# alessioGalatolo/GAN-2D-to-3D

Hardware: AMD Instinct MI355X
Metric: GAN2Shape step iters/sec, faces 128×128 b=8, 1/2/4/8 MI355X (higher is better)
Workload: dtype f32; 1 GPU; face128_n8; image_size=128, gan_size=128, n_proj_samples=8, mfma_operands=f32, prior=ellipsoid, step_mix=7:7:6 (step1:step2:step3, main.py:148 stage 0), images_per_rank=1

## Files before the change

gan-2d-to-3d_amd/csrc/conv_wgrad_core.h:

```cpp
#pragma once
#include <algorithm>
#include "g2s_common.h"

namespace g2s {

typedef float wg_f32x16 __attribute__((ext_vector_type(16)));

constexpr int WG_BM = 64, WG_BN = 64, WG_BK = 32, WG_THREADS = 256;
constexpr int WG_E = WG_BM * WG_BK / WG_THREADS;

struct WgradParams {
    const float *A, *G;
    float *dw;
    int B, Ca, Cg, PH, PW, GH, GW, k, stride, pad;
    int N;
    int K;
    int ktiles;
    int per;
    int atomic;
    int groups;
};

__device__ __forceinline__ void wgrad_block(const WgradParams &p, float (&As)[WG_BK][WG_BM + 1],
                                            float (&Bs)[WG_BK][WG_BN + 1], const int bx, const int by,
                                            const int bz) {
    const int tid = threadIdx.x, lane = tid & 63, wave = tid >> 6;
    const int wm = wave >> 1, wn = wave & 1, l31 = lane & 31, lk = lane >> 5;
    const int tiles_m = (p.Ca + WG_BM - 1) / WG_BM;
    const int m0 = (bx % tiles_m) * WG_BM, n0 = (bx / tiles_m) * WG_BN;
    const int kt0 = by * p.per, kt1 = min(p.ktiles, kt0 + p.per);
    const int P = p.PH * p.PW, KK = p.k * p.k;
    const int grp = bz;
    const int Ca_tot = p.Ca * p.groups, Cg_tot = p.Cg * p.groups;

    const int kl = tid & 31, r0 = tid >> 5;
    int gbase[WG_E], dy[WG_E], dx[WG_E];
    bool nok[WG_E], aok[WG_E];
#pragma unroll
    for (int e = 0; e < WG_E; e++) {
        const int n = n0 + r0 + 8 * e;
        nok[e] = n < p.N;
        const int g = n / KK, t = n - g * KK;
        gbase[e] = g * p.GH * p.GW;
        dy[e] = t / p.k - p.pad;
        dx[e] = t % p.k - p.pad;
        aok[e] = m0 + r0 + 8 * e < p.Ca;
    }
    float ra[WG_E], rb[WG_E];
    auto load = [&](int kt) {
        const int kg = kt * WG_BK + kl;
        const bool kok = kg < p.K;
        const int b = kok ? kg / P : 0, pix = kok ? kg - b * P : 0;
        const int py = pix / p.PW, px = pix - py * p.PW;
        const float *ap = p.A + ((size_t)b * Ca_tot + grp * p.Ca + m0 + r0) * P + pix;
        const float *gp = p.G + ((size_t)b * Cg_tot + grp * p.Cg) * p.GH * p.GW;
        const int gy0 = py * p.stride, gx0 = px * p.stride;
#pragma unroll
        for (int e = 0; e < WG_E; e++) {
            ra[e] = (kok && aok[e]) ? ap[(size_t)8 * e * P] : 0.0f;
            const int gy = gy0 + dy[e], gx = gx0 + dx[e];
            const bool ok = kok && nok[e] && gy >= 0 && gy < p.GH && gx >= 0 && gx < p.GW;
            rb[e] = ok ? gp[gbase[e] + gy * p.GW + gx] : 0.0f;
        }
    };
    wg_f32x16 acc;
#pragma unroll
    for (int r = 0; r < 16; r++) acc[r] = 0.0f;
    if (kt0 < kt1) load(kt0);
    for (int kt = kt0; kt < kt1; kt++) {
        __syncthreads();
#pragma unroll
        for (int e = 0; e < WG_E; e++) {
            As[kl][r0 + 8 * e] = ra[e];
            Bs[kl][r0 + 8 * e] = rb[e];
        }
        __syncthreads();
        if (kt + 1 < kt1) load(kt + 1);
#pragma unroll
        for (int k2 = 0; k2 < WG_BK; k2 += 2) {
            const float a = As[k2 + lk][wm * 32 + l31];
            const float b = Bs[k2 + lk][wn * 32 + l31];
            acc = __builtin_amdgcn_mfma_f32_32x32x2f32(a, b, acc, 0, 0, 0);
        }
    }
    const int n = n0 + wn * 32 + l31;
// ... 51 lines not shown
```

gan-2d-to-3d_amd/csrc/modconv.hip:

```cpp
#include "modconv_desc.h"
#include "conv_wgrad_core.h"
#include "thinconv.h"
#include "xcd_tile.h"

namespace g2s {

template <int T> struct KTile {
    static constexpr int BKT = (T == 9) ? 18 : (T == 25) ? 26 : 16;
    static constexpr int CPT = BKT / T;
    static constexpr int KMAX = (T == 25) ? 26 : 18;
};

template <int BM, int BN, int T, bool PARTIAL, bool SCALE>
__device__ __forceinline__ void modconv_body(const ConvDesc &d, const ConvClass &c,
                                             float (&As)[2][KTile<T>::KMAX][BM + 1],
                                             float (&Bs)[2][KTile<T>::KMAX + 1][BN],
                                             const int (&stab)[25], const int tile_id, const int grp,
                                             const int kt_begin, const int kt_end, const bool atomic) {
    constexpr int BKT = KTile<T>::BKT, CPT = KTile<T>::CPT, BK_MAX = KTile<T>::KMAX;
    constexpr int WAVES_M = BM >= 64 ? 2 : 1, WAVES_N = 4 / WAVES_M;
    constexpr int WMT = BM / (32 * WAVES_M), WNT = BN / (32 * WAVES_N);
    constexpr bool WIDE = (T == 9);
    constexpr int EA = WIDE ? (BM * 6 + NTHREADS - 1) / NTHREADS : (BM * BKT + NTHREADS - 1) / NTHREADS;
    constexpr int EB = (BN * BKT + NTHREADS - 1) / NTHREADS;
    const int tid = threadIdx.x, lane = tid & 63, wave = tid >> 6;
    const int wm = wave / WAVES_N, wn = wave % WAVES_N;
    const int Ncls = d.B * c.OH * c.OW;
    const int tiles_m = (d.M + BM - 1) / BM;
    const int m0 = (tile_id % tiles_m) * BM;
    const int n0 = (tile_id / tiles_m) * BN;
    const int HW = d.H * d.W;
    constexpr int OOB = 0x7fffffff;

    const auto rx = __builtin_amdgcn_make_buffer_rsrc((void *)(d.x + (size_t)grp * d.Cr * HW), 0,
                                                      (d.B * d.Cx - grp * d.Cr) * HW * 4, 0x00020000);
    const auto rw = __builtin_amdgcn_make_buffer_rsrc((void *)(d.w + (size_t)grp * (d.w_bytes / 4)), 0, d.w_bytes, 0x00020000);
    const auto rsc = __builtin_amdgcn_make_buffer_rsrc(
        (void *)(SCALE ? d.in_scale : d.w), 0, SCALE ? d.B * d.Cr * 4 : 4, 0x00020000);

    const int nB = tid % BN;
    const int ng = n0 + nB;
    const bool n_ok = ng < Ncls;
    int bb = 0, iy0 = 0, ix0 = 0;
    if (n_ok) {
        bb = ng / (c.OH * c.OW);
        const int r = ng % (c.OH * c.OW);
        iy0 = (r / c.OW) * d.is;
        ix0 = (r % c.OW) * d.is;
    }
    int offB[EB], dchB[EB];
#pragma unroll
    for (int e = 0; e < EB; e++) {
        const int k = tid / BN + e * (NTHREADS / BN);
        const int dch = k / T, t = k - dch * T;
        const int tb = stab[t < T ? t : 0];
        const int iy = iy0 + (tb & 0xff) - 8, ix = ix0 + ((tb >> 8) & 0xff) - 8;
        const bool ok = n_ok && k < BKT && dch < CPT && iy >= 0 && iy < d.H && ix >= 0 && ix < d.W;
        offB[e] = ok ? (((bb * d.Cx + dch) * d.H + iy) * d.W + ix) * 4 : OOB;
        dchB[e] = dch;
    }
    const int offS = n_ok ? bb * d.Cr * 4 : OOB;
    int offA[EA], ldsA[EA], dchA[EA];
#pragma unroll
    for (int e = 0; e < EA; e++) {
        const int idx = tid + e * NTHREADS;
        if (WIDE) {
            const int m = idx / 6, r = idx % 6, dch = r / 3, tg = r % 3;
            const bool in = idx < BM * 6, ok = in && m0 + m < d.M;
            offA[e] = ok ? ((m0 + m) * d.w_ms + dch * d.w_ks + 3 * tg) * 4 : OOB;
            ldsA[e] = in ? (dch * 9 + 3 * tg) * (BM + 1) + m : BM;
            dchA[e] = dch;
        } else {
            const int k = idx % BKT, m = idx / BKT;
            const int dch = k / T, t = k - dch * T;
            const bool ok = idx < BM * BKT && dch < CPT && m0 + m < d.M;
            offA[e] = ok ? ((m0 + m) * d.w_ms + dch * d.w_ks + (stab[t] >> 16)) * 4 : OOB;
            ldsA[e] = (idx < BM * BKT) ? k * (BM + 1) + m : BM;
            dchA[e] = dch;
        }
    }

    float ra[EA][WIDE ? 3 : 1], rb[EB];
    float rs[WIDE ? 2 : EB], rsn[2];
    auto loadA = [&](int e, int kt) {
        const int ch0 = kt * CPT;
        const int vo = (PARTIAL && dchA[e] >= d.Cr - ch0) ? OOB : offA[e];
        if constexpr (WIDE) {
            const u32x3 v = __builtin_amdgcn_raw_buffer_load_b96(rw, vo, ch0 * d.w_ks * 4, 0);
            ra[e][0] = __uint_as_float(v.x);
            ra[e][1] = __uint_as_float(v.y);
            ra[e][2] = __uint_as_float(v.z);
        } else {
            ra[e][0] = __uint_as_float(__builtin_amdgcn_raw_buffer_load_b32(rw, vo, ch0 * d.w_ks * 4, 0));
        }
    };
    auto loadB = [&](int e, int kt) {
        const int ch0 = kt * CPT;
        const bool out = PARTIAL && dchB[e] >= d.Cr - ch0;
        rb[e] = __uint_as_float(__builtin_amdgcn_raw_buffer_load_b32(rx, out ? OOB : offB[e], ch0 * HW * 4, 0));
        if constexpr (SCALE && !WIDE)
            rs[e] = __uint_as_float(__builtin_amdgcn_raw_buffer_load_b32(
                rsc, out ? OOB : offS + dchB[e] * 4, ch0 * 4, 0));
    };
    auto loadS = [&](int kt, float (&dst)[2]) {
        if constexpr (SCALE && WIDE) {
            const int ch0 = kt * CPT;
            dst[0] = __uint_as_float(__builtin_amdgcn_raw_buffer_load_b32(rsc, offS, ch0 * 4, 0));
            dst[1] = __uint_as_float(__builtin_amdgcn_raw_buffer_load_b32(
                rsc, (PARTIAL && 1 >= d.Cr - ch0) ? OOB : offS + 4, ch0 * 4, 0));
        }
    };
    auto storeA = [&](int e, float *abuf) {
        if constexpr (WIDE) {
            abuf[ldsA[e]] = ra[e][0];
            abuf[ldsA[e] + (BM + 1)] = ra[e][1];
            abuf[ldsA[e] + 2 * (BM + 1)] = ra[e][2];
        } else {
            abuf[ldsA[e]] = ra[e][0];
        }
    };
    auto storeB = [&](int e, float (*bbuf)[BN]) {
        const int k = tid / BN + e * (NTHREADS / BN);
        float v = rb[e];
        if constexpr (SCALE) v *= WIDE ? (dchB[e] ? rs[1] : rs[0]) : rs[e];
        bbuf[k < BKT ? k : BK_MAX][nB] = v;
    };

    f32x16 acc[WMT][WNT];
#pragma unroll
    for (int i = 0; i < WMT; i++)
#pragma unroll
        for (int j = 0; j < WNT; j++)
#pragma unroll
            for (int r = 0; r < 16; r++) acc[i][j][r] = 0.0f;

    const int kt_last = kt_end - 1;
#pragma unroll
    for (int e = 0; e < EA; e++) loadA(e, kt_begin);
#pragma unroll
    for (int e = 0; e < EB; e++) loadB(e, kt_begin);
    if constexpr (WIDE) loadS(kt_begin, rs);
#pragma unroll
    for (int e = 0; e < EA; e++) { storeA(e, &As[0][0][0]); loadA(e, min(kt_begin + 1, kt_last)); }
#pragma unroll
    for (int e = 0; e < EB; e++) { storeB(e, Bs[0]); loadB(e, min(kt_begin + 1, kt_last)); }
    if constexpr (WIDE) loadS(min(kt_begin + 1, kt_last), rs);
    __syncthreads();
// ... 62 lines not shown
#pragma unroll
        for (int i = 0; i < WMT; i++)
#pragma unroll
            for (int r = 0; r < 16; r++) {
                const int m = m0 + wm * (BM / WAVES_M) + i * 32 + (r & 3) + 8 * (r >> 2) + 4 * lk;
                if (m >= d.M) continue;
                float v = acc[i][j][r];
                if (ob) v *= ob[m];
                if (gbias) v += gbias[m];
                v += nz;
                if (d.act) v = (v > 0.0f ? v : v * d.act_alpha) * d.act_gain;
                float *dst = yb + (size_t)m * d.OHf * d.OWf;
                if (atomic) unsafeAtomicAdd(dst, v);
                else *dst = v;
            }
    }
}

static __host__ __device__ inline int ktiles_of(int Cr, int T) {
    const int cpt = (T == 9) ? 2 : (T == 25) ? 1 : 16 / T;
    return (Cr + cpt - 1) / cpt;
}

template <int BM, int BN, int KMAX>
__device__ __forceinline__ void modconv_segment(const ConvDesc &d, const ConvClass &c,
                                                float (&As)[2][KMAX][BM + 1], float (&Bs)[2][KMAX + 1][BN],
                                                const int (&stab)[25], const int tile_id, const int grp,
                                                const int kb, const int ke, const bool atomic) {
    const bool scale = d.in_scale != nullptr;
#define G2S_BODY(T, PART, SC) modconv_body<BM, BN, T, PART, SC>(d, c, As, Bs, stab, tile_id, grp, kb, ke, atomic)
#define G2S_TAPS(T, CPT)                                   \
    if (d.Cr % CPT) {                                      \
        if (scale) G2S_BODY(T, true, true);                \
        else G2S_BODY(T, true, false);                     \
    } else {                                               \
        if (scale) G2S_BODY(T, false, true);               \
        else G2S_BODY(T, false, false);                    \
    }
    if constexpr (KMAX == 26) {
        G2S_BODY(25, true, false);
    } else {
        switch (c.T) {
        case 9: G2S_TAPS(9, 2) break;
        case 16: G2S_BODY(16, true, false); break;
        case 4: G2S_TAPS(4, 4) break;
        case 2: G2S_TAPS(2, 8) break;
        default: G2S_TAPS(1, 16) break;
        }
    }
#undef G2S_TAPS
#undef G2S_BODY
}

template <int BM, int BN, int KMAX>
__device__ __forceinline__ void modconv_block(const ConvDesc &d, float (&As)[2][KMAX][BM + 1],
                                              float (&Bs)[2][KMAX + 1][BN], int (&stab)[25], const int nx,
                                              const int bx, const int by, const int bz, const int row) {
    const int tiles_m = (d.M + BM - 1) / BM;
    const int tile_all0 = __builtin_amdgcn_readfirstlane(xcd_logical_tile(nx, bx, row));
    const ConvClass &c = d.cls[bz];
    const int mt_all = tile_all0 % (tiles_m * d.groups);
    const int grp = __builtin_amdgcn_readfirstlane(mt_all / tiles_m);
    const int tile_id = __builtin_amdgcn_readfirstlane((tile_all0 / (tiles_m * d.groups)) * tiles_m + mt_all % tiles_m);
    if ((int)(tile_id / tiles_m) * BN >= d.B * c.OH * c.OW) return;
    const int ktiles = ktiles_of(d.Cr, c.T);
    const int slices = d.cls_splitk[bz];
    const int per = (ktiles + slices - 1) / slices;
    const int kb = by * per;
    if (by >= slices || kb >= ktiles) return;
    if (threadIdx.x < 25) stab[threadIdx.x] = c.tab[threadIdx.x];
    __syncthreads();
    modconv_segment<BM, BN, KMAX>(d, c, As, Bs, stab, tile_id, grp, kb, min(ktiles, kb + per), slices > 1);
}

template <int BM, int BN, int KMAX>
__global__ __launch_bounds__(NTHREADS) void modconv_kernel(ConvDesc d) {
    __shared__ float As[2][KMAX][BM + 1];
    __shared__ float Bs[2][KMAX + 1][BN];
    __shared__ int stab[25];
    modconv_block<BM, BN, KMAX>(d, As, Bs, stab, gridDim.x, blockIdx.x, blockIdx.y, blockIdx.z,
                                blockIdx.y + gridDim.y * blockIdx.z);
}

__global__ __launch_bounds__(NTHREADS) void conv_wgrad_rider_kernel(WgradParams p) {
    __shared__ float Wa[WG_BK][WG_BM + 1];
    __shared__ float Wb[WG_BK][WG_BN + 1];
    wgrad_block(p, Wa, Wb, blockIdx.x, blockIdx.y, blockIdx.z);
}

template <int BM, int BN, int KMAX>
__global__ __launch_bounds__(NTHREADS) void conv_bwd_kernel(ConvDesc d, WgradParams p, int nx, int ny, int n_dgrad,
                                                            int w_tiles, int w_split) {
    __shared__ float As[2][KMAX][BM + 1];
    __shared__ float Bs[2][KMAX + 1][BN];
    __shared__ int stab[25];
    __shared__ float Wa[WG_BK][WG_BM + 1];
    __shared__ float Wb[WG_BK][WG_BN + 1];
    const int lin = blockIdx.x;
    if (lin < n_dgrad) {
        const int bx = lin % nx, row = lin / nx;
        modconv_block<BM, BN, KMAX>(d, As, Bs, stab, nx, bx, row % ny, row / ny, row);
    } else {
        const int l = lin - n_dgrad;
        const int bx = l % w_tiles, r = l / w_tiles;
        wgrad_block(p, Wa, Wb, bx, r % w_split, r / w_split);
    }
}

}

using namespace g2s;

struct TunedConv { int B, Cin, Cout, H, k, mode, transpose, fused, tile, splitk; };
static const TunedConv kTuned[] = {
#include "modconv_tuned.inc"
    {0, 0, 0, 0, 0, 0, 0, 0, 0, 0}};

struct TunedConv2d { int B, Cr, M, H, k, stride, pad, adjoint, m_major, fused, groups, tile, splitk; };
static const TunedConv2d kTuned2d[] = {
#include "conv2d_tuned.inc"
    {0, 0, 0, 0, 0, 0, 0, 0, 0, 0, 0, 0, 0}};

static thread_local int g_force_tile = -1, g_force_splitk = -1;

extern "C" int g2s_modconv_tune(int tile, int splitk) {
    G2S_REQUIRE(tile >= -2 && tile <= 4 && splitk >= -1 && splitk <= 64 && splitk != 0,
                "tile must be -1 (built-in), -2 (heuristic without the tuned table) or 0..4, "
                "splitk -1 (built-in) or 1..64");
    g_force_tile = tile;
    g_force_splitk = splitk;
    return G2S_OK;
}

struct ConvGeom {
    int k, stride, pad, adjoint, m_major;
    int out_h, out_w;
};

struct WgradRider {
    WgradParams p;
    int tiles, split;
    bool dw_is_zero;
};

struct Epilogue {
    const float *bias, *noise, *noise_w;
    int act;
    float alpha, gain;
};

template <int KMAX>
static void conv_launch_tile(const ConvDesc &d, const dim3 grid, const int pick, hipStream_t st,
                             const WgradRider *rider = nullptr) {
    const int n_dgrad = grid.x * grid.y * grid.z;
#define G2S_TILE(BM_, BN_)                                                                                           \
    if (rider)                                                                                                       \
        conv_bwd_kernel<BM_, BN_, KMAX><<<n_dgrad + rider->tiles * rider->split * rider->p.groups, NTHREADS, 0, st>>>( \
            d, rider->p, grid.x, grid.y, n_dgrad, rider->tiles, rider->split);                                       \
    else                                                                                                             \
        modconv_kernel<BM_, BN_, KMAX><<<grid, NTHREADS, 0, st>>>(d)
    switch (pick) {
    case 0: modconv_kernel<128, 128, KMAX><<<grid, NTHREADS, 0, st>>>(d); break;
    case 1: modconv_kernel<128, 64, KMAX><<<grid, NTHREADS, 0, st>>>(d); break;
    case 2: G2S_TILE(64, 64); break;
    case 3: G2S_TILE(32, 128); break;
    default: G2S_TILE(64, 128); break;
    }
#undef G2S_TILE
}

static int conv_launch(const float *x, const float *w, const float *in_scale, const float *out_scale,
                       const Epilogue &ep, float *y, int B, int Cr, int M, int H, int W, const ConvGeom &g,
                       int tuned_tile, int tuned_splitk, g2s_stream_t stream, bool y_is_zero = false,
                       bool f16_operands = false, int groups = 1, const WgradRider *rider = nullptr,
                       int *plan_needs_zero = nullptr) {
    G2S_REQUIRE(plan_needs_zero || (x && w && y), "x, w, y must not be NULL");
    G2S_REQUIRE(B > 0 && Cr > 0 && M > 0 && H > 0 && W > 0, "sizes must be positive");
    const int k = g.k, s_ = g.stride, p_ = g.pad, KK = k * k;
    G2S_REQUIRE(k >= 1 && k <= 5, "kernel size must be 1..5 (got %d)", k);
    G2S_REQUIRE(s_ == 1 || s_ == 2, "stride must be 1 or 2 (got %d)", s_);
    G2S_REQUIRE(p_ >= 0 && p_ < k, "padding must be in [0, k)");
    ConvDesc d{};
    d.x = x;
    d.w = w;
    d.in_scale = in_scale;
    d.out_scale = out_scale;
    d.bias = ep.bias;
    d.noise = ep.noise;
    d.noise_w = ep.noise_w;
    G2S_REQUIRE(!d.noise || (!f16_operands && groups == 1), "the noise epilogue exists for the fp32 kernel only");
    d.act = ep.act;
// ... 65 lines not shown
        G2S_REQUIRE(!(in_scale && T > 9), "input scales are limited to kernels of up to 3x3");
        big = big || T == 25;
    }
    long nmax = 0;
    int kt_min = 1 << 30;
    for (int i = 0; i < d.ncls; i++) {
        nmax = std::max(nmax, (long)B * d.cls[i].OH * d.cls[i].OW);
        kt_min = std::min(kt_min, ktiles_of(d.Cr, d.cls[i].T));
    }
    G2S_REQUIRE(nmax < (1l << 30) && (long)B * d.Cx * H * W < (1l << 29) && (long)groups * M * Cr * KK < (1l << 29),
                "problem too large for 32-bit byte offsets");
    hipStream_t st = as_stream(stream);
    const int cfgs[5][2] = {{128, 128}, {128, 64}, {64, 64}, {32, 128}, {64, 128}};
    int pick = 2;
    for (int i = 0; i < 3; i++) {
        const long blocks = (long)groups * cdiv(d.M, cfgs[i][0]) * cdiv(nmax, cfgs[i][1]) * d.ncls;
        if (d.M > cfgs[i][0] / 2 && blocks >= 512) { pick = i; break; }
    }
    if (d.M <= 32 && nmax >= 1024 && !f16_operands) pick = 3;
    if (f16_operands && pick == 1) pick = 2;
    if (tuned_tile >= 0 && g_force_tile != -2) pick = tuned_tile;
    else tuned_splitk = -1;
    if (g_force_tile >= 0) pick = g_force_tile;
    const int BMv = cfgs[pick][0], BNv = cfgs[pick][1];
    const int tiles = groups * cdiv(d.M, BMv) * cdiv(nmax, BNv);
    int splitk = 1;
    while ((long)tiles * d.ncls * splitk < 512 && kt_min / (splitk * 2) >= 8 && splitk < 64) splitk *= 2;
    if (tuned_splitk > 0) splitk = tuned_splitk;
    if (g_force_splitk > 0) splitk = g_force_splitk;
    if (deterministic()) splitk = 1;
    splitk = std::max(1, std::min(splitk, kt_min));
    dim3 grid(tiles, splitk, d.ncls);
    const bool split = splitk > 1;
    const bool deferred_epilogue = split && (ep.bias != nullptr || ep.act != 0 || ep.noise != nullptr);
    if (deferred_epilogue) {
        d.bias = nullptr;
        d.noise = d.noise_w = nullptr;
        d.act = 0;
    }
    d.splitk = splitk;
    int kt_max = 1;
    for (int i = 0; i < d.ncls; i++) kt_max = std::max(kt_max, ktiles_of(d.Cr, d.cls[i].T));
    for (int i = 0; i < d.ncls; i++) {
        const int kt = ktiles_of(d.Cr, d.cls[i].T);
        d.cls_splitk[i] = std::max(1, std::min(kt, (int)(((long)splitk * kt + kt_max / 2) / kt_max)));
    }
    if (plan_needs_zero) {
        *plan_needs_zero = (split || holes) ? 1 : 0;
        return G2S_OK;
    }
    if ((split || holes) && !y_is_zero) {
        if (hipMemsetAsync(y, 0, (size_t)B * d.My * d.OHf * d.OWf * sizeof(float), st) != hipSuccess)
            return fail(G2S_ERR_LAUNCH, "hipMemsetAsync(y) failed");
    }
    if (f16_operands) {
        const int rc = modconv_f16_launch(d, grid, pick, st);
        if (rc != G2S_OK) return rc;
    } else if (rider) {
        const WgradParams &p = rider->p;
        if (p.atomic && !rider->dw_is_zero &&
            hipMemsetAsync(p.dw, 0, (size_t)p.groups * p.Ca * p.N * sizeof(float), st) != hipSuccess)
            return fail(G2S_ERR_LAUNCH, "hipMemsetAsync(dw) failed");
        if (big) conv_launch_tile<26>(d, grid, pick, st, pick >= 2 ? rider : nullptr);
        else conv_launch_tile<18>(d, grid, pick, st, pick >= 2 ? rider : nullptr);
        if (pick < 2) conv_wgrad_rider_kernel<<<dim3(rider->tiles, rider->split, p.groups), NTHREADS, 0, st>>>(p);
    } else if (big) {
        conv_launch_tile<26>(d, grid, pick, st);
    } else {
        conv_launch_tile<18>(d, grid, pick, st);
    }
    int rc = check_launch("g2s_modconv");
    if (rc != G2S_OK || !deferred_epilogue) return rc;
    if (ep.noise) {
        G2S_REQUIRE(ep.bias && ep.act == 1, "noise epilogue: needs a bias and act = 1");
        return g2s_noise_bias_act(y, ep.noise, ep.noise_w, ep.bias, y, B, d.My, d.OHf * d.OWf, ep.alpha, ep.gain,
                                  stream);
    }
    return g2s_fused_bias_act(y, ep.bias, nullptr, y, (int64_t)B * d.My * d.OHf * d.OWf,
                              (int64_t)d.OHf * d.OWf, d.My, ep.act ? 3 : 1, 0, ep.alpha,
                              ep.act ? ep.gain : 1.0f, G2S_F32, stream);
}

static int modconv_launch(const float *x, const float *w, const float *in_scale,
                          const float *out_scale, const Epilogue &ep, float *y, int B, int Cin, int Cout, int H,
                          int W, int k, int mode, int transpose, g2s_stream_t stream, bool f16_operands = false,
// ... 71 lines not shown
        for (const TunedConv2d *t = kTuned2d; t->B; ++t)
            if (t->B == B && t->Cr == Cr && t->M == M && t->H == H && t->k == k && t->stride == stride &&
                t->pad == pad && t->adjoint == g.adjoint && t->m_major == g.m_major &&
                t->fused == (bias != nullptr || act != 0) && t->groups == groups) {
                tile = t->tile;
                splitk = t->splitk;
                break;
            }
    return conv_launch(x, w, nullptr, nullptr, Epilogue{bias, nullptr, nullptr, act, alpha, gain}, y, B, Cr, M, H, W,
                       g, tile, splitk, stream, y_is_zero != 0, false, groups, rider);
}

extern "C" int g2s_conv2d(const float *x, const float *w, const float *bias, float *y, int B, int Cr, int M, int H,
                          int W, int k, int stride, int pad, int adjoint, int w_m_major, int out_h, int out_w, int act,
                          float alpha, float gain, int y_is_zero, int groups, g2s_stream_t stream) {
    return conv2d_impl(x, w, bias, y, B, Cr, M, H, W, k, stride, pad, adjoint, w_m_major, out_h, out_w, act, alpha,
                       gain, y_is_zero, groups, stream);
}

extern "C" int g2s_conv2d_bwd(const float *gy, const float *w, float *gx, int B, int Cr, int M, int H, int W, int k,
                              int stride, int pad, int adjoint, int w_m_major, int out_h, int out_w, int gx_is_zero,
                              const float *A, const float *G, float *dw, int Ca, int Cg, int PH, int PW, int GH,
                              int GW, int dw_is_zero, int groups, g2s_stream_t stream) {
    WgradRider rider;
    const int rc = wgrad_plan(A, G, dw, B, Ca, Cg, PH, PW, GH, GW, k, stride, pad, groups, rider.p, rider.tiles,
                              rider.split);
    if (rc != G2S_OK) return rc;
    rider.dw_is_zero = dw_is_zero != 0;
    return conv2d_impl(gy, w, nullptr, gx, B, Cr, M, H, W, k, stride, pad, adjoint, w_m_major, out_h, out_w, 0, 0.0f,
                       1.0f, gx_is_zero, groups, stream, &rider);
}
```

gan-2d-to-3d_amd/lib.py:

```python
import ctypes as C
import os

import torch

_HERE = os.path.dirname(os.path.abspath(__file__))
LIB_PATH = os.path.join(_HERE, "lib", "libg2s.so")

G2S_F32, G2S_F16 = 0, 1
CONV_PLAIN, CONV_UP2, CONV_DOWN2 = 0, 1, 2

_lib = None

_p, _i, _f, _sz, _i64, _d = C.c_void_p, C.c_int, C.c_float, C.c_size_t, C.c_int64, C.c_double
SIGNATURES = {
    "g2s_abi_version": (_i, []),
    "g2s_last_error": (C.c_char_p, []),
    "g2s_clamp": (_i, [_p, _p, _p, _i64, _f, _f, _i, _p]),
    "g2s_avg_pyramid": (_i, [_p, _p, _i, _i64, _i, _i, _p]),
    "g2s_res_split_fwd": (_i, [_p, _p, _p, _i64, _i, _i, _p]),
    "g2s_res_split_bwd": (_i, [_p, _p, _p, _p, _i64, _i, _i, _p]),
    "g2s_depth_head_fwd": (_i, [_p, _p, _p, _i64, _i, _f, _f, _i, _f, _p]),
    "g2s_depth_head_bwd": (_i, [_p, _p, _p, _p, _p, _i64, _i, _f, _f, _i, _f, _i, _p]),
    "g2s_grid_sample_fwd": (_i, [_p, _p, _p, _i, _i, _i, _i, _i, _i, _i, _f, _f, _p]),
    "g2s_grid_sample_bwd_workspace_bytes": (_sz, [_i, _i, _i, _i]),
# ... 16 lines not shown
    "g2s_noise_bias_act": (_i, [_p, _p, _p, _p, _p, _i, _i, _i, _f, _f, _p]),
    "g2s_upfirdn2d": (_i, [_p, _p, _p] + [_i] * 14 + [_p]),
    "g2s_modconv": (_i, [_p] * 8 + [_i] * 9 + [_f, _f, _i, _p]),
    "g2s_modconv_needs_zero": (_i, [_i, _i, _i, _i, _i, _i, _i, _i, _i, _i]),
    "g2s_upfirdn2d_nba": (_i, [_p, _p, _p] + [_i] * 12 + [_p, _p, _p, _f, _f, _p]),
    "g2s_synth_bwd_rows": (_i, [_p] * 13 + [_i, _i, _i, _f, _f, _p]),
    "g2s_channel_sum": (_i, [_p, _p, _i, _i, _i, _p]),
    "g2s_demod_fwd_multi": (_i, [_p, _p, _p, _p, _p, _i, _i, _f, _p]),
    "g2s_demod_bwd_multi": (_i, [_p, _p, _p, _p, _p, _p, _p, _i, _i, _p]),
    "g2s_modconv_f16": (_i, [_p, _p, _p, _p, _p, _p, _i, _i, _i, _i, _i, _i, _i, _i, _i, _f, _f, _p]),
    "g2s_modconv_tune": (_i, [_i, _i]),
    "g2s_mfma_probe": (_i, [_p, _i, _i, _i, _p]),
    "g2s_mfma_lds_probe": (_i, [_p, _i, _i, _i, _i, _p]),
    "g2s_wino_weights_floats": (_sz, [_i, _i]),
    "g2s_wino4_weights_floats": (_sz, [_i, _i]),
    "g2s_wino4_weights": (_i, [_p, _p, _i, _i, _i, _p]),
    "g2s_wino4_supported": (_i, [_i] * 5),
    "g2s_conv3x3_wino4": (_i, [_p] * 8 + [_i] * 6 + [_f, _f, _i, _p, _i64, _p]),
    "g2s_wino_weights": (_i, [_p, _p, _i, _i, _i, _p]),
    "g2s_conv3x3_wino": (_i, [_p] * 8 + [_i] * 6 + [_f, _f, _i, _p, _i64, _p]),
    "g2s_conv2d": (_i, [_p, _p, _p, _p] + [_i] * 12 + [_i, _f, _f, _i, _i, _p]),
    "g2s_conv2d_wgrad": (_i, [_p, _p, _p] + [_i] * 10 + [_i, _i, _p]),
    "g2s_conv2d_bwd": (_i, [_p, _p, _p] + [_i] * 13 + [_p, _p, _p] + [_i] * 8 + [_p]),
    "g2s_adam_chunk": (_i64, []),
    "g2s_adam_step": (_i, [_p, _p, _p, _i, _i, _f, _f, _f, _f, _f, _p]),
    "g2s_rows_dot_scale": (_i, [_p, _p, _p, _p, _p, _p, _i, _i, _p]),
    "g2s_demod_fwd": (_i, [_p, _p, _p, _i, _i, _i, _f, _p]),
    "g2s_demod_bwd": (_i, [_p, _p, _p, _p, _p, _i, _i, _i, _p]),
    "g2s_demod_bwd_add": (_i, [_p, _p, _p, _p, _p, _p, _i, _i, _i, _p]),
    "g2s_lpips_layer_fwd": (_i, [_p, _p, _p, _p, _i, _i, _i, _p]),
    "g2s_lpips_layer_bwd": (_i, [_p, _p, _p, _p, _p, _i, _i, _i, _p]),
    "g2s_lpips_layer_bwd_ex": (_i, [_p, _p, _p, _p, _p, _i, _p, _i, _i, _i, _p]),
    "g2s_weighted_l1_fwd": (_i, [_p, _p, _p, _p, _i, _i, _i, _p]),
    "g2s_weighted_l1_bwd": (_i, [_p, _p, _p, _p, _p, _i, _i, _i, _p]),
    "g2s_weighted_l1_fwd2": (_i, [_p, _p, _p, _p, _i, _i, _i, _p]),
    "g2s_weighted_l1_bwd3": (_i, [_p] * 7 + [_f, _p, _p, _f, _f, _p, _i, _i, _i, _p]),
    "g2s_weighted_l1_bwd2": (_i, [_p, _p, _p, _p, _p, _p, _p, _i, _i, _i, _p]),
    "g2s_view_transform_fwd": (_i, [_p, _f, _f, _f, _p, _p, _i, _p]),
    "g2s_view_transform_bwd": (_i, [_p, _f, _f, _f, _p, _p, _p, _i, _p]),
    "g2s_warp_verts_fwd": (_i, [_p, _p, _p, _p, _f, _p, _i, _i, _p]),
    "g2s_warp_verts_bwd": (_i, [_p, _p, _p, _p, _f, _p, _p, _i, _i, _i, _p]),
    "g2s_inv_warp_grid_fwd": (_i, [_p, _p, _p, _p, _p, _f, _p, _i, _i, _i, _p]),
    "g2s_inv_warp_grid_bwd": (_i, [_p, _p, _p, _p, _p, _f, _p, _p, _p, _i, _i, _i, _i, _p]),
    "g2s_normal_fwd": (_i, [_p, _p, _p, _i, _i, _i, _p]),
    "g2s_normal_bwd": (_i, [_p, _p, _p, _p, _i, _i, _i, _p]),
    "g2s_shading_fwd": (_i, [_p, _p, _p, _p, _p, _i, _i, _i, _i, _p]),
# ... 74 lines not shown
```

gan-2d-to-3d_amd/op/conv.py:

```python
import torch
from torch.autograd import Function

from gan2shape_amd import lib as _lib
from gan2shape_amd import zeropool


class PassArena:

    LIMIT = 1 << 20

    def __init__(self, device, fwd_elems):
        self.device = device
        self.fwd = zeropool.zeros(fwd_elems, device) if fwd_elems else None
        self.fwd_off = 0
        self.bwd_need = 0
        self.bwd = None
        self.bwd_off = 0

    @staticmethod
    def _pad(n):
        return (n + 63) & ~63

    def take_fwd(self, shape):
        n = 1
# ... 64 lines not shown


def _conv_bwd_raw(gy, w, x, cin, cout, k, stride, pad, transposed, gx_out=None, gw_out=None, groups=1):
    B, _, H, W = gy.shape
    oh, ow = x.shape[2], x.shape[3]
    adjoint = not transposed
    gx = gx_out if gx_out is not None else torch.empty((B, groups * cin, oh, ow), dtype=torch.float32, device=gy.device)
    A, G = (x, gy) if transposed else (gy, x)
    Ca, Cg = A.shape[1] // groups, G.shape[1] // groups
    dw = gw_out if gw_out is not None else torch.empty((groups * Ca, Cg, k, k), dtype=torch.float32, device=gy.device)
    L = _lib.load()
    from gan2shape_amd.modconv import profiled
    sp = H * W if adjoint else oh * ow
    flop = 2.0 * B * groups * cout * cin * k * k * sp + 2.0 * B * groups * Ca * Cg * k * k * A.shape[2] * A.shape[3]
    with profiled(flop, 4.0 * (2 * gy.numel() + w.numel() + gx.numel() + x.numel() + dw.numel())):
        _lib.check(L.g2s_conv2d_bwd(_lib.ptr(gy), _lib.ptr(w), _lib.ptr(gx), B, cout, cin, H, W, k, stride, pad,
                                    int(adjoint), int(transposed), oh if adjoint else 0, ow if adjoint else 0,
                                    int(gx_out is not None), _lib.ptr(A), _lib.ptr(G), _lib.ptr(dw), Ca, Cg,
                                    A.shape[2], A.shape[3], G.shape[2], G.shape[3], int(gw_out is not None),
                                    groups, _lib.stream()))
    return gx, dw


class ConvFunction(Function):

    @staticmethod
    def forward(ctx, x, w, bias, stride, pad, transposed, slope, arena=None, groups=1):
        _lib.require_cuda(x, w, bias)
        if x.dtype != torch.float32 or w.dtype != torch.float32:
            raise RuntimeError("conv: float32 only")
        x, w = x.contiguous(), w.contiguous()
        k = w.shape[2]
        cin, cout = (w.shape[0] // groups, w.shape[1]) if transposed else (w.shape[1], w.shape[0] // groups)
        if x.shape[1] != groups * cin:
            raise RuntimeError(f"conv: input has {x.shape[1]} channels, weight expects {groups * cin}")
        if groups != 1 and bias is not None:
            raise RuntimeError("grouped conv: no bias")
        b = None if bias is None else bias.contiguous()
        out = None
        if arena is not None:
            oh, ow = _out_size(x.shape[2], x.shape[3], k, stride, pad, transposed)
            out = arena.take_fwd((x.shape[0], groups * cout, oh, ow))
            if ctx.needs_input_grad[0]:
                arena.reserve_bwd(x.numel())
            if ctx.needs_input_grad[1]:
                arena.reserve_bwd(w.numel())
        y = _conv2d_raw(x, w, b, cin, cout, k, stride, pad, transposed, not transposed, None,
                        slope is not None, slope or 0.0, out=out, groups=groups)
        ctx.save_for_backward(x, w, y if slope is not None else None)
        ctx.cfg = (stride, pad, transposed, slope, bias is not None, groups)
        ctx.arena = arena
        return y

    @staticmethod
    def backward(ctx, gy):
        x, w, y = ctx.saved_tensors
        stride, pad, transposed, slope, has_bias, groups = ctx.cfg
        k = w.shape[2]
        gy = gy.contiguous()
        if slope is not None:
            from gan2shape_amd.plugins import fused
            gy = fused.fused_bias_act(gy, gy.new_empty(0), y, 3, 1, float(slope), 1.0)
        cin, cout = (w.shape[0] // groups, w.shape[1]) if transposed else (w.shape[1], w.shape[0] // groups)
        gx = gw = gb = None
        arena = ctx.arena
        if ctx.needs_input_grad[0] and ctx.needs_input_grad[1]:
            gx_out = None if arena is None else arena.take_bwd(tuple(x.shape))
            gw_out = None if arena is None else arena.take_bwd(tuple(w.shape))
            gx, gw = _conv_bwd_raw(gy, w, x, cin, cout, k, stride, pad, transposed, gx_out, gw_out, groups)
        elif ctx.needs_input_grad[0]:
            out = None if arena is None else arena.take_bwd(tuple(x.shape))
            gx = _conv2d_raw(gy, w, None, cout, cin, k, stride, pad, not transposed, transposed,
                             (x.shape[2], x.shape[3]), False, 0.0, out=out, groups=groups)
        elif ctx.needs_input_grad[1]:
            out = None if arena is None else arena.take_bwd(tuple(w.shape))
            gw = (_wgrad(x, gy, k, stride, pad, out, groups) if transposed
                  else _wgrad(gy, x, k, stride, pad, out, groups))
        if has_bias and ctx.needs_input_grad[2]:
            gb = torch.empty(gy.shape[1], dtype=torch.float32, device=gy.device)
            _lib.check(_lib.load().g2s_channel_sum(_lib.ptr(gy), _lib.ptr(gb), gy.shape[0], gy.shape[1],
                                                   gy.shape[2] * gy.shape[3], _lib.stream()))
        return gx, gw, gb, None, None, None, None, None, None
# ... 43 lines not shown
```

include/g2s.h:

```cpp
#ifndef G2S_H
#define G2S_H

#include <stddef.h>
#include <stdint.h>

#ifdef __cplusplus
extern "C" {
#endif

#define G2S_ABI_VERSION 1

#define G2S_OK 0
#define G2S_ERR_INVALID (-1)
#define G2S_ERR_LAUNCH (-2)
#define G2S_ERR_WORKSPACE (-3)

#define G2S_F32 0
#define G2S_F16 1

typedef void *g2s_stream_t;

int g2s_abi_version(void);
const char *g2s_last_error(void);

// ... 83 lines not shown



#define G2S_CONV_PLAIN 0
#define G2S_CONV_UP2 1
#define G2S_CONV_DOWN2 2

int g2s_modconv(const float *x, const float *w, const float *in_scale, const float *out_scale, const float *bias,
                const float *noise, const float *noise_w, float *y, int B, int Cin, int Cout, int H, int W, int k,
                int mode, int transpose, int act, float alpha, float gain, int y_is_zero, g2s_stream_t stream);
int g2s_modconv_needs_zero(int B, int Cin, int Cout, int H, int W, int k, int mode, int transpose,
                           int has_scales, int fused);

int g2s_conv2d(const float *x, const float *w, const float *bias, float *y, int B, int Cr, int M, int H,
               int W, int k, int stride, int pad, int adjoint, int w_m_major, int out_h, int out_w,
               int act, float alpha, float gain, int y_is_zero, int groups, g2s_stream_t stream);
int g2s_conv2d_wgrad(const float *A, const float *G, float *dw, int B, int Ca, int Cg, int PH, int PW,
                     int GH, int GW, int k, int stride, int pad, int dw_is_zero, int groups, g2s_stream_t stream);

int g2s_conv2d_bwd(const float *gy, const float *w, float *gx, int B, int Cr, int M, int H, int W, int k,
                   int stride, int pad, int adjoint, int w_m_major, int out_h, int out_w, int gx_is_zero,
                   const float *A, const float *G, float *dw, int Ca, int Cg, int PH, int PW, int GH, int GW,
                   int dw_is_zero, int groups, g2s_stream_t stream);

#define G2S_ADAM_MAX_TENSORS 128
typedef struct g2s_adam_tensor {
    float *p, *m, *v;
    int64_t n;
    float *step;
    int *ticket;
} g2s_adam_tensor;
int64_t g2s_adam_chunk(void);
int g2s_adam_step(const g2s_adam_tensor *tensors, const int *chunk0, const float *const *grads, int n_tensors,
                  int n_chunks, float lr, float beta1, float beta2, float eps, float weight_decay,
                  g2s_stream_t stream);

int g2s_modconv_f16(const float *x, const float *w, const float *in_scale, const float *out_scale,
                    const float *bias, float *y, int B, int Cin, int Cout, int H, int W, int k, int mode,
                    int transpose, int act, float alpha, float gain, g2s_stream_t stream);

size_t g2s_wino_weights_floats(int M, int Cr);
int g2s_wino_weights(const float *w, float *U, int Cout, int Cin, int transpose, g2s_stream_t stream);
int g2s_conv3x3_wino(const float *x, const float *U, const float *in_scale, const float *out_scale,
                     const float *bias, const float *noise, const float *noise_w, float *y, int B, int Cr, int M,
                     int H, int W, int act, float alpha, float gain, int splitk, float *ws, int64_t ws_floats,
                     g2s_stream_t stream);
// ... 105 lines not shown
```

Before: 206.2 iters/s.

## Fuse conv backward (leaky-ReLU gate, dgrad, wgrad, bias grad) into one launch

Adds g2s_conv2d_layer_bwd, which applies the leaky-ReLU gradient gate inline while loading gy in the dgrad, wgrad and new bias-reduction blocks, all dispatched from a single conv_bwd_kernel launch. It replaces the separate fused_bias_act gate pass, the materialized gated gy, and separate bias-grad work in ConvFunction.backward, which is enabled by default. In exchange the gate reference is re-read inside each sub-kernel, small-tile picks are forced to a rider-capable tile, and bias grads use atomics when sliced.

Measured after the change: 201.1 iters/s. 2.5% lower.

```diff
diff --git a/gan-2d-to-3d_amd/csrc/conv_wgrad_core.h b/gan-2d-to-3d_amd/csrc/conv_wgrad_core.h
--- a/gan-2d-to-3d_amd/csrc/conv_wgrad_core.h
+++ b/gan-2d-to-3d_amd/csrc/conv_wgrad_core.h
@@ -21,9 +21,13 @@
     int groups;
 };
 
+__device__ __forceinline__ float gate_factor(const float ref, const float slope) { return ref > 0.0f ? 1.0f : slope; }
+
+template <bool GATE = false>
 __device__ __forceinline__ void wgrad_block(const WgradParams &p, float (&As)[WG_BK][WG_BM + 1],
                                             float (&Bs)[WG_BK][WG_BN + 1], const int bx, const int by,
-                                            const int bz) {
+                                            const int bz, const float *ref = nullptr, const float slope = 0.0f,
+                                            const bool gate_g = false) {
     const int tid = threadIdx.x, lane = tid & 63, wave = tid >> 6;
     const int wm = wave >> 1, wn = wave & 1, l31 = lane & 31, lk = lane >> 5;
     const int tiles_m = (p.Ca + WG_BM - 1) / WG_BM;
@@ -52,8 +56,10 @@
         const bool kok = kg < p.K;
         const int b = kok ? kg / P : 0, pix = kok ? kg - b * P : 0;
         const int py = pix / p.PW, px = pix - py * p.PW;
-        const float *ap = p.A + ((size_t)b * Ca_tot + grp * p.Ca + m0 + r0) * P + pix;
-        const float *gp = p.G + ((size_t)b * Cg_tot + grp * p.Cg) * p.GH * p.GW;
+        const size_t ao = ((size_t)b * Ca_tot + grp * p.Ca + m0 + r0) * P + pix;
+        const size_t go = ((size_t)b * Cg_tot + grp * p.Cg) * p.GH * p.GW;
+        const float *ap = p.A + ao;
+        const float *gp = p.G + go;
         const int gy0 = py * p.stride, gx0 = px * p.stride;
 #pragma unroll
         for (int e = 0; e < WG_E; e++) {
@@ -61,6 +67,13 @@
             const int gy = gy0 + dy[e], gx = gx0 + dx[e];
             const bool ok = kok && nok[e] && gy >= 0 && gy < p.GH && gx >= 0 && gx < p.GW;
             rb[e] = ok ? gp[gbase[e] + gy * p.GW + gx] : 0.0f;
+            if constexpr (GATE) {
+                if (gate_g) {
+                    if (ok) rb[e] *= gate_factor(ref[go + gbase[e] + gy * p.GW + gx], slope);
+                } else {
+                    if (kok && aok[e]) ra[e] *= gate_factor(ref[ao + (size_t)8 * e * P], slope);
+                }
+            }
         }
     };
     wg_f32x16 acc;
diff --git a/gan-2d-to-3d_amd/csrc/modconv.hip b/gan-2d-to-3d_amd/csrc/modconv.hip
--- a/gan-2d-to-3d_amd/csrc/modconv.hip
+++ b/gan-2d-to-3d_amd/csrc/modconv.hip
@@ -11,8 +11,13 @@
     static constexpr int KMAX = (T == 25) ? 26 : 18;
 };
 
-template <int BM, int BN, int T, bool PARTIAL, bool SCALE>
-__device__ __forceinline__ void modconv_body(const ConvDesc &d, const ConvClass &c,
+struct Gate {
+    const float *ref;
+    float slope;
+};
+
+template <int BM, int BN, int T, bool PARTIAL, bool SCALE, bool GATE>
+__device__ __forceinline__ void modconv_body(const ConvDesc &d, const ConvClass &c, const Gate &gate,
                                              float (&As)[2][KTile<T>::KMAX][BM + 1],
                                              float (&Bs)[2][KTile<T>::KMAX + 1][BN],
                                              const int (&stab)[25], const int tile_id, const int grp,
@@ -37,6 +42,9 @@
     const auto rw = __builtin_amdgcn_make_buffer_rsrc((void *)(d.w + (size_t)grp * (d.w_bytes / 4)), 0, d.w_bytes, 0x00020000);
     const auto rsc = __builtin_amdgcn_make_buffer_rsrc(
         (void *)(SCALE ? d.in_scale : d.w), 0, SCALE ? d.B * d.Cr * 4 : 4, 0x00020000);
+    const auto rgate = __builtin_amdgcn_make_buffer_rsrc(
+        (void *)(GATE ? gate.ref + (size_t)grp * d.Cr * HW : d.w), 0, GATE ? (d.B * d.Cx - grp * d.Cr) * HW * 4 : 4,
+        0x00020000);
 
     const int nB = tid % BN;
     const int ng = n0 + nB;
@@ -82,6 +90,7 @@
 
     float ra[EA][WIDE ? 3 : 1], rb[EB];
     float rs[WIDE ? 2 : EB], rsn[2];
+    float rg[GATE ? EB : 1];
     auto loadA = [&](int e, int kt) {
         const int ch0 = kt * CPT;
         const int vo = (PARTIAL && dchA[e] >= d.Cr - ch0) ? OOB : offA[e];
@@ -101,6 +110,8 @@
         if constexpr (SCALE && !WIDE)
             rs[e] = __uint_as_float(__builtin_amdgcn_raw_buffer_load_b32(
                 rsc, out ? OOB : offS + dchB[e] * 4, ch0 * 4, 0));
+        if constexpr (GATE)
+            rg[e] = __uint_as_float(__builtin_amdgcn_raw_buffer_load_b32(rgate, out ? OOB : offB[e], ch0 * HW * 4, 0));
     };
     auto loadS = [&](int kt, float (&dst)[2]) {
         if constexpr (SCALE && WIDE) {
@@ -123,6 +134,7 @@
         const int k = tid / BN + e * (NTHREADS / BN);
         float v = rb[e];
         if constexpr (SCALE) v *= WIDE ? (dchB[e] ? rs[1] : rs[0]) : rs[e];
+        if constexpr (GATE) v *= gate_factor(rg[e], gate.slope);
         bbuf[k < BKT ? k : BK_MAX][nB] = v;
     };
 
@@ -231,19 +243,20 @@
     return (Cr + cpt - 1) / cpt;
 }
 
-template <int BM, int BN, int KMAX>
-__device__ __forceinline__ void modconv_segment(const ConvDesc &d, const ConvClass &c,
+template <int BM, int BN, int KMAX, bool GATE>
+__device__ __forceinline__ void modconv_segment(const ConvDesc &d, const ConvClass &c, const Gate &gate,
                                                 float (&As)[2][KMAX][BM + 1], float (&Bs)[2][KMAX + 1][BN],
                                                 const int (&stab)[25], const int tile_id, const int grp,
                                                 const int kb, const int ke, const bool atomic) {
-    const bool scale = d.in_scale != nullptr;
-#define G2S_BODY(T, PART, SC) modconv_body<BM, BN, T, PART, SC>(d, c, As, Bs, stab, tile_id, grp, kb, ke, atomic)
+    const bool scale = !GATE && d.in_scale != nullptr;
+#define G2S_BODY(T, PART, SC) \
+    modconv_body<BM, BN, T, PART, SC, GATE>(d, c, gate, As, Bs, stab, tile_id, grp, kb, ke, atomic)
 #define G2S_TAPS(T, CPT)                                   \
     if (d.Cr % CPT) {                                      \
-        if (scale) G2S_BODY(T, true, true);                \
+        if (scale) G2S_BODY(T, true, !GATE);               \
         else G2S_BODY(T, true, false);                     \
     } else {                                               \
-        if (scale) G2S_BODY(T, false, true);               \
+        if (scale) G2S_BODY(T, false, !GATE);              \
         else G2S_BODY(T, false, false);                    \
     }
     if constexpr (KMAX == 26) {
@@ -261,10 +274,11 @@
 #undef G2S_BODY
 }
 
-template <int BM, int BN, int KMAX>
+template <int BM, int BN, int KMAX, bool GATE = false>
 __device__ __forceinline__ void modconv_block(const ConvDesc &d, float (&As)[2][KMAX][BM + 1],
                                               float (&Bs)[2][KMAX + 1][BN], int (&stab)[25], const int nx,
-                                              const int bx, const int by, const int bz, const int row) {
+                                              const int bx, const int by, const int bz, const int row,
+                                              const Gate &gate = Gate{nullptr, 0.0f}) {
     const int tiles_m = (d.M + BM - 1) / BM;
     const int tile_all0 = __builtin_amdgcn_readfirstlane(xcd_logical_tile(nx, bx, row));
     const ConvClass &c = d.cls[bz];
@@ -279,7 +293,7 @@
     if (by >= slices || kb >= ktiles) return;
     if (threadIdx.x < 25) stab[threadIdx.x] = c.tab[threadIdx.x];
     __syncthreads();
-    modconv_segment<BM, BN, KMAX>(d, c, As, Bs, stab, tile_id, grp, kb, min(ktiles, kb + per), slices > 1);
+    modconv_segment<BM, BN, KMAX, GATE>(d, c, gate, As, Bs, stab, tile_id, grp, kb, min(ktiles, kb + per), slices > 1);
 }
 
 template <int BM, int BN, int KMAX>
@@ -297,9 +311,41 @@
     wgrad_block(p, Wa, Wb, blockIdx.x, blockIdx.y, blockIdx.z);
 }
 
-template <int BM, int BN, int KMAX>
-__global__ __launch_bounds__(NTHREADS) void conv_bwd_kernel(ConvDesc d, WgradParams p, int nx, int ny, int n_dgrad,
-                                                            int w_tiles, int w_split) {
+struct BwdTail {
+    const float *gate_ref;
+    float slope;
+    int gate_g;
+    const float *gy;
+    float *gb;
+    int B, C, P;
+    int slices, per;
+};
+
+template <bool GATE>
+__device__ __forceinline__ void bias_grad_block(const BwdTail &t, float *red, const int l) {
+    const int c = l % t.C, i0 = (l / t.C) * t.per, i1 = min(t.B * t.P, i0 + t.per);
+    float sum = 0.0f;
+    for (int i = i0 + (int)threadIdx.x; i < i1; i += NTHREADS) {
+        const int b = i / t.P;
+        const size_t o = ((size_t)b * t.C + c) * t.P + (i - b * t.P);
+        float v = t.gy[o];
+        if constexpr (GATE) v *= gate_factor(t.gate_ref[o], t.slope);
+        sum += v;
+    }
+#pragma unroll
+    for (int o = 32; o > 0; o >>= 1) sum += __shfl_down(sum, o, 64);
+    if ((threadIdx.x & 63) == 0) red[threadIdx.x >> 6] = sum;
+    __syncthreads();
+    if (threadIdx.x == 0) {
+        const float r = red[0] + red[1] + red[2] + red[3];
+        if (t.slices > 1) unsafeAtomicAdd(t.gb + c, r);
+        else t.gb[c] = r;
+    }
+}
+
+template <int BM, int BN, int KMAX, bool GATE>
+__global__ __launch_bounds__(NTHREADS) void conv_bwd_kernel(ConvDesc d, WgradParams p, BwdTail t, int nx, int ny,
+                                                            int n_dgrad, int n_wgrad, int w_tiles, int w_split) {
     __shared__ float As[2][KMAX][BM + 1];
     __shared__ float Bs[2][KMAX + 1][BN];
     __shared__ int stab[25];
@@ -308,11 +354,13 @@
     const int lin = blockIdx.x;
     if (lin < n_dgrad) {
         const int bx = lin % nx, row = lin / nx;
-        modconv_block<BM, BN, KMAX>(d, As, Bs, stab, nx, bx, row % ny, row / ny, row);
-    } else {
+        modconv_block<BM, BN, KMAX, GATE>(d, As, Bs, stab, nx, bx, row % ny, row / ny, row, Gate{t.gate_ref, t.slope});
+    } else if (lin < n_dgrad + n_wgrad) {
         const int l = lin - n_dgrad;
         const int bx = l % w_tiles, r = l / w_tiles;
-        wgrad_block(p, Wa, Wb, bx, r % w_split, r / w_split);
+        wgrad_block<GATE>(p, Wa, Wb, bx, r % w_split, r / w_split, t.gate_ref, t.slope, t.gate_g != 0);
+    } else {
+        bias_grad_block<GATE>(t, &Wa[0][0], lin - n_dgrad - n_wgrad);
     }
 }
 
@@ -350,6 +398,11 @@
     WgradParams p;
     int tiles, split;
     bool dw_is_zero;
+    BwdTail tail;
+    bool gb_is_zero;
+    bool has_tail() const { return tail.gate_ref != nullptr || tail.gb != nullptr; }
+    int n_wgrad() const { return tiles * split * p.groups; }
+    int n_bias() const { return tail.gb ? tail.C * tail.slices : 0; }
 };
 
 struct Epilogue {
@@ -362,12 +415,13 @@
 static void conv_launch_tile(const ConvDesc &d, const dim3 grid, const int pick, hipStream_t st,
                              const WgradRider *rider = nullptr) {
     const int n_dgrad = grid.x * grid.y * grid.z;
-#define G2S_TILE(BM_, BN_)                                                                                           \
-    if (rider)                                                                                                       \
-        conv_bwd_kernel<BM_, BN_, KMAX><<<n_dgrad + rider->tiles * rider->split * rider->p.groups, NTHREADS, 0, st>>>( \
-            d, rider->p, grid.x, grid.y, n_dgrad, rider->tiles, rider->split);                                       \
-    else                                                                                                             \
-        modconv_kernel<BM_, BN_, KMAX><<<grid, NTHREADS, 0, st>>>(d)
+#define G2S_BWD(BM_, BN_, GATE_)                                                                              \
+    conv_bwd_kernel<BM_, BN_, KMAX, GATE_><<<n_dgrad + rider->n_wgrad() + rider->n_bias(), NTHREADS, 0, st>>>( \
+        d, rider->p, rider->tail, grid.x, grid.y, n_dgrad, rider->n_wgrad(), std::max(1, rider->tiles), rider->split)
+#define G2S_TILE(BM_, BN_)                                           \
+    if (rider && rider->tail.gate_ref) G2S_BWD(BM_, BN_, true);      \
+    else if (rider) G2S_BWD(BM_, BN_, false);                        \
+    else modconv_kernel<BM_, BN_, KMAX><<<grid, NTHREADS, 0, st>>>(d)
     switch (pick) {
     case 0: modconv_kernel<128, 128, KMAX><<<grid, NTHREADS, 0, st>>>(d); break;
     case 1: modconv_kernel<128, 64, KMAX><<<grid, NTHREADS, 0, st>>>(d); break;
@@ -376,6 +430,18 @@
     default: G2S_TILE(64, 128); break;
     }
 #undef G2S_TILE
+#undef G2S_BWD
+}
+
+static int rider_clear(const WgradRider &r, hipStream_t st) {
+    const WgradParams &p = r.p;
+    if (r.tiles && p.atomic && !r.dw_is_zero &&
+        hipMemsetAsync(p.dw, 0, (size_t)p.groups * p.Ca * p.N * sizeof(float), st) != hipSuccess)
+        return fail(G2S_ERR_LAUNCH, "hipMemsetAsync(dw) failed");
+    if (r.tail.gb && r.tail.slices > 1 && !r.gb_is_zero &&
+        hipMemsetAsync(r.tail.gb, 0, (size_t)r.tail.C * sizeof(float), st) != hipSuccess)
+        return fail(G2S_ERR_LAUNCH, "hipMemsetAsync(gb) failed");
+    return G2S_OK;
 }
 
 static int conv_launch(const float *x, const float *w, const float *in_scale, const float *out_scale,
@@ -487,6 +553,7 @@
     if (tuned_tile >= 0 && g_force_tile != -2) pick = tuned_tile;
     else tuned_splitk = -1;
     if (g_force_tile >= 0) pick = g_force_tile;
+    if (rider && rider->has_tail() && pick < 2) pick = 4;
     const int BMv = cfgs[pick][0], BNv = cfgs[pick][1];
     const int tiles = groups * cdiv(d.M, BMv) * cdiv(nmax, BNv);
     int splitk = 1;
@@ -523,9 +590,8 @@
         if (rc != G2S_OK) return rc;
     } else if (rider) {
         const WgradParams &p = rider->p;
-        if (p.atomic && !rider->dw_is_zero &&
-            hipMemsetAsync(p.dw, 0, (size_t)p.groups * p.Ca * p.N * sizeof(float), st) != hipSuccess)
-            return fail(G2S_ERR_LAUNCH, "hipMemsetAsync(dw) failed");
+        const int rc_clear = rider_clear(*rider, st);
+        if (rc_clear != G2S_OK) return rc_clear;
         if (big) conv_launch_tile<26>(d, grid, pick, st, pick >= 2 ? rider : nullptr);
         else conv_launch_tile<18>(d, grid, pick, st, pick >= 2 ? rider : nullptr);
         if (pick < 2) conv_wgrad_rider_kernel<<<dim3(rider->tiles, rider->split, p.groups), NTHREADS, 0, st>>>(p);
@@ -643,7 +709,7 @@
                               int stride, int pad, int adjoint, int w_m_major, int out_h, int out_w, int gx_is_zero,
                               const float *A, const float *G, float *dw, int Ca, int Cg, int PH, int PW, int GH,
                               int GW, int dw_is_zero, int groups, g2s_stream_t stream) {
-    WgradRider rider;
+    WgradRider rider{};
     const int rc = wgrad_plan(A, G, dw, B, Ca, Cg, PH, PW, GH, GW, k, stride, pad, groups, rider.p, rider.tiles,
                               rider.split);
     if (rc != G2S_OK) return rc;
@@ -651,3 +717,47 @@
     return conv2d_impl(gy, w, nullptr, gx, B, Cr, M, H, W, k, stride, pad, adjoint, w_m_major, out_h, out_w, 0, 0.0f,
                        1.0f, gx_is_zero, groups, stream, &rider);
 }
+
+extern "C" int g2s_conv2d_layer_bwd(const float *gy, const float *gate_ref, float slope, const float *w, float *gx,
+                                    int B, int Cr, int M, int H, int W, int k, int stride, int pad, int adjoint,
+                                    int w_m_major, int out_h, int out_w, int gx_is_zero, const float *A,
+                                    const float *G, float *dw, int Ca, int Cg, int PH, int PW, int GH, int GW,
+                                    int dw_is_zero, float *gb, int gb_is_zero, int groups, g2s_stream_t stream) {
+    G2S_REQUIRE(gy && (gx || dw || gb), "gy and at least one of gx, dw, gb must not be NULL");
+    G2S_REQUIRE(B > 0 && Cr > 0 && H > 0 && W > 0 && groups >= 1 && groups <= 8, "sizes must be positive, groups 1..8");
+    G2S_REQUIRE((long)B * groups * Cr * H * W < (1l << 29), "gy too large for 32-bit byte offsets");
+    G2S_REQUIRE(!gate_ref || (slope == slope && slope - slope == 0.0f), "slope must be finite");
+    WgradRider rider{};
+    rider.split = 1;
+    rider.p.groups = groups;
+    if (dw) {
+        G2S_REQUIRE(A == gy || G == gy, "one weight-gradient operand must be gy");
+        const int rc = wgrad_plan(A, G, dw, B, Ca, Cg, PH, PW, GH, GW, k, stride, pad, groups, rider.p, rider.tiles,
+                                  rider.split);
+        if (rc != G2S_OK) return rc;
+        G2S_REQUIRE(G == gy ? (Cg == Cr && GH == H && GW == W) : (Ca == Cr && PH == H && PW == W),
+                    "the gy operand of the weight gradient must have the shape of gy");
+    }
+    rider.dw_is_zero = dw_is_zero != 0;
+    rider.gb_is_zero = gb_is_zero != 0;
+    BwdTail &t = rider.tail;
+    t.gate_ref = gate_ref;
+    t.slope = slope;
+    t.gate_g = G == gy;
+    t.gy = gy;
+    t.gb = gb;
+    t.B = B;
+    t.C = groups * Cr;
+    t.P = H * W;
+    t.slices = deterministic() ? 1 : std::max(1, std::min(cdiv((long)B * t.P, 2048), 512 / t.C));
+    t.per = cdiv((long)B * t.P, t.slices);
+    t.slices = cdiv((long)B * t.P, t.per);
+    if (gx)
+        return conv2d_impl(gy, w, nullptr, gx, B, Cr, M, H, W, k, stride, pad, adjoint, w_m_major, out_h, out_w, 0,
+                           0.0f, 1.0f, gx_is_zero, groups, stream, &rider);
+    hipStream_t st = as_stream(stream);
+    const int rc = rider_clear(rider, st);
+    if (rc != G2S_OK) return rc;
+    conv_launch_tile<18>(ConvDesc{}, dim3(0, 1, 1), 2, st, &rider);
+    return check_launch("g2s_conv2d_layer_bwd");
+}
diff --git a/gan-2d-to-3d_amd/lib.py b/gan-2d-to-3d_amd/lib.py
--- a/gan-2d-to-3d_amd/lib.py
+++ b/gan-2d-to-3d_amd/lib.py
@@ -62,6 +62,7 @@
     "g2s_conv2d": (_i, [_p, _p, _p, _p] + [_i] * 12 + [_i, _f, _f, _i, _i, _p]),
     "g2s_conv2d_wgrad": (_i, [_p, _p, _p] + [_i] * 10 + [_i, _i, _p]),
     "g2s_conv2d_bwd": (_i, [_p, _p, _p] + [_i] * 13 + [_p, _p, _p] + [_i] * 8 + [_p]),
+    "g2s_conv2d_layer_bwd": (_i, [_p, _p, _f, _p, _p] + [_i] * 13 + [_p, _p, _p] + [_i] * 7 + [_p, _i, _i, _p]),
     "g2s_adam_chunk": (_i64, []),
     "g2s_adam_step": (_i, [_p, _p, _p, _i, _i, _f, _f, _f, _f, _f, _p]),
     "g2s_rows_dot_scale": (_i, [_p, _p, _p, _p, _p, _p, _i, _i, _p]),
diff --git a/gan-2d-to-3d_amd/op/conv.py b/gan-2d-to-3d_amd/op/conv.py
--- a/gan-2d-to-3d_amd/op/conv.py
+++ b/gan-2d-to-3d_amd/op/conv.py
@@ -110,7 +110,42 @@
     return gx, dw
 
 
+def _layer_bwd_raw(gy, y, slope, w, x, cin, cout, k, stride, pad, transposed, want_gx, want_gw, want_gb,
+                   gx_out=None, gw_out=None, gb_out=None, groups=1):
+    B, C, H, W = gy.shape
+    oh, ow = x.shape[2], x.shape[3]
+    adjoint = not transposed
+    dev = gy.device
+    gx = gw = gb = None
+    if want_gx:
+        gx = gx_out if gx_out is not None else torch.empty((B, groups * cin, oh, ow), dtype=torch.float32, device=dev)
+    A, G = (x, gy) if transposed else (gy, x)
+    Ca, Cg = A.shape[1] // groups, G.shape[1] // groups
+    if want_gw:
+        gw = gw_out if gw_out is not None else torch.empty((groups * Ca, Cg, k, k), dtype=torch.float32, device=dev)
+    if want_gb:
+        gb = gb_out if gb_out is not None else torch.empty(C, dtype=torch.float32, device=dev)
+    L = _lib.load()
+    from gan2shape_amd.modconv import profiled
+    sp = H * W if adjoint else oh * ow
+    flop = ((2.0 * B * groups * cout * cin * k * k * sp if want_gx else 0.0)
+            + (2.0 * B * groups * Ca * Cg * k * k * A.shape[2] * A.shape[3] if want_gw else 0.0))
+    reads = (int(want_gx) + int(want_gw) + int(want_gb)) * gy.numel() * (2 if y is not None else 1)
+    moved = (reads + (w.numel() + gx.numel() if want_gx else 0) + (x.numel() + gw.numel() if want_gw else 0)
+             + (C if want_gb else 0))
+    with profiled(flop, 4.0 * moved):
+        _lib.check(L.g2s_conv2d_layer_bwd(
+            _lib.ptr(gy), _lib.ptr(y), float(slope or 0.0), _lib.ptr(w), _lib.ptr(gx), B, cout, cin, H, W, k, stride,
+            pad, int(adjoint), int(transposed), oh if adjoint else 0, ow if adjoint else 0, int(gx_out is not None),
+            _lib.ptr(A) if want_gw else None, _lib.ptr(G) if want_gw else None, _lib.ptr(gw), Ca, Cg,
+            A.shape[2], A.shape[3], G.shape[2], G.shape[3], int(gw_out is not None), _lib.ptr(gb),
+            int(gb_out is not None), groups, _lib.stream()))
+    return gx, gw, gb
+
+
 class ConvFunction(Function):
+
+    ONE_LAUNCH_BACKWARD = True
 
     @staticmethod
     def forward(ctx, x, w, bias, stride, pad, transposed, slope, arena=None, groups=1):
@@ -133,6 +168,8 @@
                 arena.reserve_bwd(x.numel())
             if ctx.needs_input_grad[1]:
                 arena.reserve_bwd(w.numel())
+            if bias is not None and ctx.needs_input_grad[2]:
+                arena.reserve_bwd(bias.numel())
         y = _conv2d_raw(x, w, b, cin, cout, k, stride, pad, transposed, not transposed, None,
                         slope is not None, slope or 0.0, out=out, groups=groups)
         ctx.save_for_backward(x, w, y if slope is not None else None)
@@ -146,6 +183,20 @@
         stride, pad, transposed, slope, has_bias, groups = ctx.cfg
         k = w.shape[2]
         gy = gy.contiguous()
+        cin, cout = (w.shape[0] // groups, w.shape[1]) if transposed else (w.shape[1], w.shape[0] // groups)
+        want_gx, want_gw = ctx.needs_input_grad[0], ctx.needs_input_grad[1]
+        want_gb = has_bias and ctx.needs_input_grad[2]
+        arena = ctx.arena
+        if ConvFunction.ONE_LAUNCH_BACKWARD and (want_gx or want_gw or want_gb):
+            def take(shape):
+                return None if arena is None else arena.take_bwd(shape)
+            gx_out = take(tuple(x.shape)) if want_gx else None
+            gw_out = take(tuple(w.shape)) if want_gw else None
+            gb_out = (take((gy.shape[1],)) if arena is not None else zeropool.take((gy.shape[1],), gy.device)) \
+                if want_gb else None
+            gx, gw, gb = _layer_bwd_raw(gy, y, slope, w, x, cin, cout, k, stride, pad, transposed, want_gx, want_gw,
+                                        want_gb, gx_out, gw_out, gb_out, groups)
+            return gx, gw, gb, None, None, None, None, None, None
         if slope is not None:
             from gan2shape_amd.plugins import fused
             gy = fused.fused_bias_act(gy, gy.new_empty(0), y, 3, 1, float(slope), 1.0)
diff --git a/include/g2s.h b/include/g2s.h
--- a/include/g2s.h
+++ b/include/g2s.h
@@ -129,6 +129,12 @@
                    int stride, int pad, int adjoint, int w_m_major, int out_h, int out_w, int gx_is_zero,
                    const float *A, const float *G, float *dw, int Ca, int Cg, int PH, int PW, int GH, int GW,
                    int dw_is_zero, int groups, g2s_stream_t stream);
+
+int g2s_conv2d_layer_bwd(const float *gy, const float *gate_ref, float slope, const float *w, float *gx, int B,
+                         int Cr, int M, int H, int W, int k, int stride, int pad, int adjoint, int w_m_major,
+                         int out_h, int out_w, int gx_is_zero, const float *A, const float *G, float *dw, int Ca,
+                         int Cg, int PH, int PW, int GH, int GW, int dw_is_zero, float *gb, int gb_is_zero,
+                         int groups, g2s_stream_t stream);
 
 #define G2S_ADAM_MAX_TENSORS 128
 typedef struct g2s_adam_tensor {
```
